# Fro116/RecommenderSystem

Measured on AMD Instinct MI355X. Metric: interactions/sec, higher is better.
Workload: dtype bf16

## Files before the change

include/rsys_debug.h:

```cpp
#ifndef RSYS_DEBUG_H
#define RSYS_DEBUG_H
#include "rsys.h"

#ifdef __cplusplus
extern "C" {
#endif

int32_t rsys_debug_get(rsys_model* m, const char* key, void* out, int64_t bytes);

int32_t rsys_local_group_create(int32_t world, int32_t device, void** group);
int32_t rsys_local_group_destroy(void* group);
int32_t rsys_comm_init_local(void* group, int32_t rank, rsys_comm** out);
int32_t rsys_comm_debug_delay(rsys_comm* c, int32_t microseconds);

int32_t rsys_dev_alloc(void** p, size_t bytes);
int32_t rsys_dev_free(void* p);
int32_t rsys_dev_h2d(void* dst, const void* src, size_t bytes);
int32_t rsys_dev_d2h(void* dst, const void* src, size_t bytes);
int32_t rsys_dev_memset(void* dst, int value, size_t bytes);
int32_t rsys_op_gemm(int32_t dtype, const void* A, const void* B, void* C, int32_t M, int32_t N, int32_t K,
                     int64_t lda, int64_t ldb, int64_t ldc, int32_t a_km, int32_t b_km, int32_t a_f32, int32_t c_f32,
                     int32_t splitk);
int32_t rsys_op_gemm_rows(int32_t dtype, const void* A, const void* B, void* C, int32_t M, int32_t N, int32_t K,
                          int64_t lda, int64_t ldb, int64_t ldc, int32_t b_km, int32_t c_f32, const int32_t* rows_dev);
// ... 7 lines not shown
int32_t rsys_debug_gemm_route(int32_t dtype, int32_t M, int32_t N, int32_t K, int64_t lda, int64_t ldb, int64_t ldc, int32_t a_km,
                              int32_t b_km, int32_t a_f32, int32_t c_f32, int32_t epi, int32_t splitk, int32_t flags, float alpha,
                              int32_t accum, int32_t set, int32_t m_expect, int32_t cus, char* tag, int32_t tag_bytes, int32_t* splits);
int32_t rsys_op_attention(int32_t dtype, int32_t B, int32_t T, int32_t H, int32_t KV, int32_t hd, const void* qkv,
                          const int32_t* uid, const int32_t* tm, void* O, float* lse, const void* dO, void* dqkv,
                          const float* rope_cos, const float* rope_sin);
int32_t rsys_op_attention_ex(int32_t dtype, int32_t B, int32_t T, int32_t H, int32_t KV, int32_t hd, const void* qkv,
                             const int32_t* uid, const int32_t* tm, void* O, float* lse, const void* dO, void* dqkv,
                             const float* rope_cos, const float* rope_sin, const int32_t* rope_pos, int32_t rope_rows,
                             const int32_t* q_active, float* amax_fwd, float* amax_bwd);
int32_t rsys_op_attention_cached(int32_t dtype, int32_t rows, int32_t T, int32_t H, int32_t KV, int32_t hd, const void* qkv, const void* cache,
                                 int32_t n_slots, const int32_t* slot, const int32_t* n_hist, const int32_t* n_cand, void* O);
int32_t rsys_op_attention_cached_tiles(int32_t dtype, int32_t rows, int32_t T, int32_t H, int32_t KV, int32_t hd, const void* qkv, const void* cache,
                                       int32_t n_slots, int32_t Tc, int32_t n_seg, const int32_t* seg, void* O);
int32_t rsys_op_rank_cache_copy_segments(int32_t dtype, int32_t rows, int32_t T, int32_t H, int32_t KV, int32_t hd, const void* qkv, void* cache,
                                         int32_t n_slots, int32_t Tc, int32_t n_seg, const int32_t* seg);
int32_t rsys_rank_cache_get(rsys_model* m, int32_t layer, int32_t slot, void* out, int64_t bytes);
int32_t rsys_op_topk(const float* scores, int64_t ld, int32_t rows, int32_t V, int32_t k,
                     int32_t* ids, float* vals, int32_t* counts);
int32_t rsys_op_target_rank(const float* scores, int64_t ld, int32_t rows, int32_t V, const int32_t* targets, int32_t* rank_out);
int32_t rsys_op_pair_ranks(const float* scores, int64_t ld, int32_t rows, int32_t V, const int32_t* self, const int64_t* tgt_offsets,
                           const int32_t* tgt_ids, int32_t* ranks_out);
int32_t rsys_sim_pair_scores(void* h, int32_t n_src, const int32_t* sources, float* out);
int32_t rsys_rank_gram_get(rsys_model* m, int32_t medium, int32_t n_groups, const int64_t* cand_offsets, const int32_t* cand_ids,
                           float* out, int64_t n_out);
int32_t rsys_op_rerank(int32_t n, int32_t partialk, const float* pen, const float* r, const float* gram, const int32_t* ss_bits,
                       const int32_t* related_bits, int32_t* picks);
int32_t rsys_render_debug_keep(rsys_model* m, int32_t on);
int32_t rsys_render_debug_get(rsys_model* m, const char* key, void* out, int64_t cap, int64_t* bytes);
int32_t rsys_sim_debug_get(void* h, const char* name, void* out, int64_t n);
int32_t rsys_search_debug_get(void* h, const char* name, float* out, int64_t n);
int32_t rsys_op_embedding_scatter(const float* gx0, int64_t ldx, const int32_t* matchedid, const int32_t* m_matchedid, int32_t N,
                                  int32_t V, int32_t D, float* gE, int32_t atomic);
int32_t rsys_op_f8_quantize(const void* src, int64_t ld_src, int32_t rows, int32_t cols, int32_t fmt, int32_t layout, int32_t seg_cols,
                            int32_t seg_rep, void* dst, int64_t ld_dst, float* amax_dev, float* desc_dev, const float* wamax_dev,
                            int32_t n_w, int32_t w_rep, int32_t desc_mode);
int32_t rsys_op_f8_weights(const float* src, int64_t ld, int32_t rows, int32_t cols, int32_t layout, int32_t seg_rows, int32_t seg_rep,
                           float* amax_dev, void* dst, void* dst_t, int64_t ld_t);
int32_t rsys_op_gemm_f8(const void* A8, const void* B8, void* C, int32_t M, int32_t N, int32_t K, int64_t lda, int64_t ldb, int64_t ldc,
                        int32_t a_fmt, int32_t c_f32, const float* desc_dev, int32_t seg_cols, int32_t alt, int32_t kb0, int32_t kb1,
                        int32_t kb2);
int32_t rsys_op_rmsnorm_fwd(int32_t dtype, const float* x, const float* scale, void* y, float* rstd, int64_t rows, int32_t D,
                            const int32_t* rows_dev, const int32_t* in_rows, float* amax);
int32_t rsys_op_rmsnorm_bwd(int32_t dtype, int32_t g_f32, const void* g, const float* x, const float* scale, const float* rstd,
                            const float* resid, const int32_t* resid_slot, const int32_t* io_rows, const int32_t* rows_dev,
                            float* dx, void* dx_t, float* dscale, int64_t rows, int32_t D, float* amax, int32_t deterministic);
int32_t rsys_op_ce(int32_t dtype, void* logits, int64_t ldl, int32_t n, int32_t V, const int32_t* idx, const float* label,
                   const float* weight, const int32_t* position, const float* stats, const int32_t* npos, float task_w, float* loss,
                   int32_t deterministic);
int32_t rsys_op_rating_tail(int32_t dtype, void* z, const void* hact, int32_t n, int32_t D, const float* w2, const float* b2,
                            const int32_t* idx, const float* label, const float* weight, const float* stats, float rating_mean,
                            float task_w, int32_t evaluate, float* loss, float* dw2, float* db2, float* db0, const int32_t* npos,
                            int32_t deterministic);
int32_t rsys_op_sumsq(const float* g, int64_t n, float* out);
int32_t rsys_op_clip_adamw(int32_t dtype, float* p, float* g, float* m, float* v, void* shadow, int64_t n_decay, int64_t n_total,
                           float lr, float b1, float b2, float eps, float wd, int32_t step, float max_norm, float grad_div,
                           int32_t zero_grad, int64_t sh_skip_lo, int64_t sh_skip_hi, int32_t fused, float* sumsq);
int32_t rsys_op_adapter_bank(int32_t dtype, int32_t stages, int32_t train, int32_t rows, int32_t Ttok, int32_t D, int32_t H, int32_t KV, int32_t hd,
                             int32_t L, int32_t layer, float p, uint64_t seed, int64_t stream, const int32_t* row_slot, const void* bankA,
                             const void* bankB, const void* xn, void* La, void* qkv, const void* dqkv, void* dLa, void* dxn, float* partA, float* partB,
                             float* gA, float* gB, const float* rope_cos, const float* rope_sin, const int32_t* rope_pos, int32_t rope_rows);
int32_t rsys_op_adapter_bank_tiles(int32_t dtype, int32_t stages, int32_t rows, int32_t Ttok, int32_t D, int32_t H, int32_t KV, int32_t hd, int32_t L,
                                   int32_t layer, const int32_t* tile_slot, const void* bankA, const void* bankB, const void* xn, void* La, void* qkv,
                                   const float* rope_cos, const float* rope_sin, const int32_t* rope_pos, int32_t rope_rows);
int32_t rsys_op_adapter_bank_segments(int32_t dtype, int32_t stages, int32_t train, int32_t rows, int32_t Ttok, int32_t D, int32_t H, int32_t KV, int32_t hd,
                                      int32_t L, int32_t layer, float p, uint64_t seed, int64_t stream, const int32_t* segs, int32_t n_seg, const void* bankA,
                                      const void* bankB, const void* xn, void* La, void* qkv, const void* dqkv, void* dLa, void* dxn, float* partA,
                                      float* partB, float* gA, float* gB, const float* rope_cos, const float* rope_sin, const int32_t* rope_pos,
                                      int32_t rope_rows);
int32_t rsys_op_adapter_bank_adamw(int32_t dtype, float* A32, float* B32, float* gA, float* gB, float* mA, float* vA, float* mB, float* vB, void* A,
                                   void* B, int64_t nA, int64_t nB, const float* per_slot, float b1, float b2, float eps, float wd, float* norms);
int32_t rsys_op_dropout(int32_t dtype, const void* src, void* dst, int64_t n, float p, uint64_t seed, int64_t stream, int32_t accumulate);
int32_t rsys_op_vp_ce(int32_t dtype, int32_t stages, int32_t deterministic, const int32_t* idx, const float* label, const float* weight,
                      const int32_t* position, const float* stats, const int32_t* npos, float task_w, int32_t KB, int32_t KBmax, float* own,
                      const void* EwAll, const float* metaAll, int32_t W, int32_t D, void* EwC, float* metaC, int32_t* nlive, int32_t* pre,
                      void* logits, int64_t ldl, int32_t Vloc, int32_t col0, float* lmax, const float* gmax, float* sums, int32_t cap,
                      int32_t rank, float* loss, int32_t rows, int32_t rows_finish);
int32_t rsys_op_ss(int32_t dtype, int32_t stages, int32_t deterministic, int32_t len, int32_t n_s, int32_t n_tot, int32_t col0, uint64_t seed,
                   int64_t stream, int32_t* cols, int32_t* bitmap, int32_t* tlist, int32_t* tcount, const float* metaC, const int32_t* nlive,
                   const int32_t* pre, int32_t rank, int32_t cap_rows, int32_t rows, int32_t rows_finish, const void* EwC, const void* Floc,
                   int32_t D, void* logits, int64_t ldl, float* lmax, float* lsum, float* tl, float* gmax, float* loss, float* dt,
                   float* gE_loc, float* dEwC, const int32_t* ridx, int32_t rbase, int64_t rld, int32_t rn, int32_t rtable_rows,
                   const void* gsrc, void* gdst, const float* asrc, float* adst);
int32_t rsys_op_shard_rows(int32_t stages, const int32_t* skey, const int32_t* sidx, int32_t N, int32_t V, int32_t* slot, int32_t* uniq,
                           int32_t* tok2u, int32_t* plan, const int32_t* bound, int32_t nb, int32_t* off, float* table, int64_t ld,
                           int32_t table_rows, const int32_t* ids, int32_t sub, float* packed, int32_t n, int32_t D, const int32_t* count,
                           const int32_t* m_matchedid, const int32_t* userid, const int32_t* m_tmid, int32_t Ntok, const float* Frem,
                           int32_t frem_rows, float* x0, int32_t* uid_t, int32_t* tm_t);

#ifdef __cplusplus
}
#endif
#endif
```

recommendersystem_amd/_lib.py:

```python
import ctypes as C
import os

os.environ.setdefault("HSA_ENABLE_IPC_MODE_LEGACY", "0")

HERE = os.path.dirname(os.path.abspath(__file__))
LIB_PATH = os.path.join(HERE, "librsys_hip.so")


class RsysError(RuntimeError):
    pass


class rsys_config(C.Structure):
    _fields_ = [
        ("num_layers", C.c_int32), ("num_heads", C.c_int32), ("num_kv_heads", C.c_int32),
        ("embed_dim", C.c_int32), ("intermediate_dim", C.c_int32), ("max_sequence_length", C.c_int32),
        ("vocab_0", C.c_int32), ("vocab_1", C.c_int32),
        ("vocab_status", C.c_int32), ("vocab_gender", C.c_int32), ("vocab_source", C.c_int32),
        ("metadata_dim", C.c_int32),
        ("min_ts", C.c_double), ("max_ts", C.c_double),
        ("rating_mean", C.c_float), ("rating_std", C.c_float), ("mask_rate", C.c_float),
        ("mask_topk", C.c_int32), ("finetune", C.c_int32), ("finetune_metric", C.c_int32),
        ("dtype", C.c_int32), ("max_rows", C.c_int32), ("lora_dropout", C.c_float),
        ("table_shard_rank", C.c_int32), ("table_shard_world", C.c_int32), ("sampled_negatives", C.c_int32),
# ... 148 lines not shown
    ("rsys_comm_init", C.c_int32, [C.POINTER(C.c_uint8 * 128), C.c_int32, C.c_int32, C.c_int32, C.POINTER(_P)]),
    ("rsys_comm_destroy", C.c_int32, [_P]),
    ("rsys_comm_debug_delay", C.c_int32, [_P, C.c_int32]),
    ("rsys_set_grad_sync", C.c_int32, [_P, _P]),
    ("rsys_model_set_split_table_reduce", C.c_int32, [_P, C.c_int32]),
    ("rsys_model_set_shard_comm", C.c_int32, [_P, _P]),
    ("rsys_table_rows", C.c_int32, [_P, C.POINTER(C.c_int64), C.POINTER(C.c_int64)]),
    ("rsys_local_group_create", C.c_int32, [C.c_int32, C.c_int32, C.POINTER(_P)]),
    ("rsys_local_group_destroy", C.c_int32, [_P]),
    ("rsys_comm_init_local", C.c_int32, [_P, C.c_int32, C.POINTER(_P)]),
    ("rsys_allreduce_grads", C.c_int32, [_P, _P]),
    ("rsys_grad_sync_early", C.c_int32, [_P, C.POINTER(C.c_int64)]),
    ("rsys_grad_sync_schedule", C.c_int32, [_P, C.POINTER(C.c_int64), C.c_int32, C.POINTER(C.c_int32)]),
    ("rsys_comm_info", C.c_int32, [_P, C.POINTER(C.c_int32)]),
    ("rsys_allreduce_f64", C.c_int32, [_P, C.POINTER(C.c_double), C.c_int32]),
    ("rsys_self_test", C.c_int32, [_P]),
    ("rsys_param_checksum", C.c_int32, [_P, C.POINTER(C.c_double * 4)]),
    ("rsys_grad_buffer", C.c_int32, [_P, C.POINTER(_P), C.POINTER(C.c_int64)]),
    ("rsys_param_buffer", C.c_int32, [_P, C.POINTER(_P), C.POINTER(C.c_int64)]),
    ("rsys_refresh_shadow", C.c_int32, [_P]),
    ("rsys_dev_alloc", C.c_int32, [C.POINTER(_P), C.c_size_t]),
    ("rsys_dev_free", C.c_int32, [_P]),
    ("rsys_dev_h2d", C.c_int32, [_P, _P, C.c_size_t]),
    ("rsys_dev_d2h", C.c_int32, [_P, _P, C.c_size_t]),
    ("rsys_dev_memset", C.c_int32, [_P, C.c_int, C.c_size_t]),
    ("rsys_op_gemm", C.c_int32, [C.c_int32, _P, _P, _P, C.c_int32, C.c_int32, C.c_int32, C.c_int64, C.c_int64, C.c_int64,
                                 C.c_int32, C.c_int32, C.c_int32, C.c_int32, C.c_int32]),
    ("rsys_op_f8_quantize", C.c_int32, [_P, C.c_int64, C.c_int32, C.c_int32, C.c_int32, C.c_int32, C.c_int32, C.c_int32, _P, C.c_int64, _P, _P, _P,
                                          C.c_int32, C.c_int32, C.c_int32]),
    ("rsys_op_f8_weights", C.c_int32, [_P, C.c_int64, C.c_int32, C.c_int32, C.c_int32, C.c_int32, C.c_int32, _P, _P, _P, C.c_int64]),
    ("rsys_op_gemm_f8", C.c_int32, [_P, _P, _P, C.c_int32, C.c_int32, C.c_int32, C.c_int64, C.c_int64, C.c_int64, C.c_int32, C.c_int32, _P,
                                      C.c_int32, C.c_int32, C.c_int32, C.c_int32, C.c_int32]),
    ("rsys_op_gemm_rows", C.c_int32, [C.c_int32, _P, _P, _P, C.c_int32, C.c_int32, C.c_int32, C.c_int64, C.c_int64, C.c_int64,
                                      C.c_int32, C.c_int32, _P]),
    ("rsys_op_gemm_klimit", C.c_int32, [C.c_int32, _P, _P, _P, C.c_int32, C.c_int32, C.c_int32, C.c_int64, C.c_int64, C.c_int64, C.c_int32, _P]),
    ("rsys_op_gemm_epi", C.c_int32, [C.c_int32, _P, _P, _P, C.c_int32, C.c_int32, C.c_int32, C.c_int64, C.c_int64, C.c_int64, C.c_int32, C.c_int32,
                                     C.c_int32, C.c_float, C.c_int32, _P, _P, C.c_int64, _P, C.c_int64, _P, _P, _P, _P, _P,
                                     C.c_int32, C.c_int32, C.c_int32, C.c_int32, _P, C.c_char_p, C.c_int32, C.POINTER(C.c_int32)]),
    ("rsys_debug_gemm_route", C.c_int32, [C.c_int32] * 4 + [C.c_int64] * 3 + [C.c_int32] * 7 + [C.c_float] + [C.c_int32] * 4
                                          + [C.c_char_p, C.c_int32, C.POINTER(C.c_int32)]),
    ("rsys_op_attention", C.c_int32, [C.c_int32] + [C.c_int32] * 5 + [_P] * 9),
    ("rsys_op_attention_ex", C.c_int32, [C.c_int32] + [C.c_int32] * 5 + [_P] * 10 + [C.c_int32, _P, _P, _P]),
    ("rsys_op_topk", C.c_int32, [_P, C.c_int64, C.c_int32, C.c_int32, C.c_int32, _P, _P, _P]),
    ("rsys_op_target_rank", C.c_int32, [_P, C.c_int64, C.c_int32, C.c_int32, _P, _P]),
    ("rsys_op_pair_ranks", C.c_int32, [_P, C.c_int64, C.c_int32, C.c_int32, _P, _P, _P, _P]),
    ("rsys_rank_gram_get", C.c_int32, [_P, C.c_int32, C.c_int32, _P, _P, _P, C.c_int64]),
    ("rsys_op_rerank", C.c_int32, [C.c_int32, C.c_int32, _P, _P, _P, _P, _P, _P]),
    ("rsys_op_embedding_scatter", C.c_int32, [_P, C.c_int64, _P, _P, C.c_int32, C.c_int32, C.c_int32, _P, C.c_int32]),
    ("rsys_op_rmsnorm_fwd", C.c_int32, [C.c_int32, _P, _P, _P, _P, C.c_int64, C.c_int32, _P, _P, _P]),
    ("rsys_op_rmsnorm_bwd", C.c_int32, [C.c_int32, C.c_int32] + [_P] * 11 + [C.c_int64, C.c_int32, _P, C.c_int32]),
    ("rsys_op_ce", C.c_int32, [C.c_int32, _P, C.c_int64, C.c_int32, C.c_int32] + [_P] * 6 + [C.c_float, _P, C.c_int32]),
    ("rsys_op_rating_tail", C.c_int32, [C.c_int32, _P, _P, C.c_int32, C.c_int32] + [_P] * 6 + [C.c_float, C.c_float, C.c_int32]
                                        + [_P] * 5 + [C.c_int32]),
    ("rsys_op_sumsq", C.c_int32, [_P, C.c_int64, _P]),
    ("rsys_op_clip_adamw", C.c_int32, [C.c_int32] + [_P] * 5 + [C.c_int64, C.c_int64] + [C.c_float] * 5
                                       + [C.c_int32, C.c_float, C.c_float, C.c_int32, C.c_int64, C.c_int64, C.c_int32, _P]),
    ("rsys_op_adapter_bank", C.c_int32, [C.c_int32] * 11 + [C.c_float, C.c_uint64, C.c_int64] + [_P] * 16 + [C.c_int32]),
    ("rsys_op_adapter_bank_tiles", C.c_int32, [C.c_int32] * 10 + [_P] * 9 + [C.c_int32]),
    ("rsys_op_adapter_bank_segments", C.c_int32, [C.c_int32] * 11 + [C.c_float, C.c_uint64, C.c_int64, _P, C.c_int32] + [_P] * 15 + [C.c_int32]),
    ("rsys_op_adapter_bank_adamw", C.c_int32, [C.c_int32] + [_P] * 10 + [C.c_int64, C.c_int64, _P] + [C.c_float] * 4 + [_P]),
    ("rsys_op_dropout", C.c_int32, [C.c_int32, _P, _P, C.c_int64, C.c_float, C.c_uint64, C.c_int64, C.c_int32]),
    ("rsys_op_vp_ce", C.c_int32, [C.c_int32] * 3 + [_P] * 6 + [C.c_float, C.c_int32, C.c_int32, _P, _P, _P, C.c_int32, C.c_int32]
                                  + [_P] * 5 + [C.c_int64, C.c_int32, C.c_int32, _P, _P, _P, C.c_int32, C.c_int32, _P, C.c_int32, C.c_int32]),
    ("rsys_op_ss", C.c_int32, [C.c_int32] * 7 + [C.c_uint64, C.c_int64] + [_P] * 7 + [C.c_int32] * 4 + [_P, _P, C.c_int32, _P, C.c_int64]
                               + [_P] * 9 + [C.c_int32, C.c_int64, C.c_int32, C.c_int32] + [_P] * 4),
    ("rsys_op_shard_rows", C.c_int32, [C.c_int32, _P, _P, C.c_int32, C.c_int32] + [_P] * 5 + [C.c_int32, _P, _P, C.c_int64, C.c_int32, _P,
                                       C.c_int32, _P, C.c_int32, C.c_int32] + [_P] * 4 + [C.c_int32, _P, C.c_int32, _P, _P, _P]),
    ("rsys_step_mark", C.c_int32, [_P]),
    ("rsys_step_marks_get", C.c_int32, [_P, _P, C.c_int32, C.POINTER(C.c_int32)]),
    ("rsys_op_timing", C.c_int32, [_P, C.c_int32]),
    ("rsys_timing_get", C.c_int32, [_P, C.c_char_p, C.c_size_t]),
    ("rsys_op_timing_filter", C.c_int32, [_P, C.c_char_p]),
    ("rsys_switches_reload", C.c_int32, []),
    ("rsys_switches_describe", C.c_int32, [C.c_char_p, C.c_int32]),
]
EXPORTED = [s[0] for s in _SIGS]

_lib = None


def lib():
    global _lib
    if _lib is None:
        if not os.path.exists(LIB_PATH):
            raise RsysError(f"{LIB_PATH} is missing: build it with `make -C recommendersystem_amd/csrc` "
                            "(there is no CPU fallback for the HIP path)")
        L = C.CDLL(LIB_PATH, mode=C.RTLD_GLOBAL)
        for name, res, args in _SIGS:
            fn = getattr(L, name)
            fn.restype = res
            fn.argtypes = args
        _lib = L
    return _lib


def last_error():
    buf = C.create_string_buffer(2048)
    lib().rsys_last_error(buf, 2048)
    return buf.value.decode(errors="replace")


def check(rc):
    if rc != 0:
        raise RsysError(f"rsys error {rc}: {last_error()}")


# ... 17 lines not shown
```

recommendersystem_amd/csrc/capi.hip:

```cpp
#include <algorithm>
#include <dlfcn.h>
#include <math.h>
#include <stdlib.h>
#include <string.h>

#include <sstream>

#include "comm.hpp"
#include "encoder_handle.hpp"
#include "model_internal.hpp"

namespace rsys {
static thread_local std::string g_err;
void set_error(const std::string& msg) { g_err = msg; }
}

using namespace rsys;

struct rsys_model { Model* m; };
struct rsys_optimizer { Optimizer o; };

#define CHECK_HANDLE(h) do { if ((h) == nullptr) { set_error("null handle"); return RSYS_ERR_ARG; } } while (0)

extern "C" {
// ... 1136 lines not shown
int32_t rsys_op_rmsnorm_bwd(int32_t dtype, int32_t g_f32, const void* g, const float* x, const float* scale, const float* rstd,
                            const float* resid, const int32_t* resid_slot, const int32_t* io_rows, const int32_t* rows_dev,
                            float* dx, void* dx_t, float* dscale, int64_t rows, int32_t D, float* amax, int32_t deterministic) {
  switches_parse();
  ARG_CHECK(g && x && scale && rstd && dx && dscale && rows >= 0, "rsys_op_rmsnorm_bwd: arguments");
  ARG_CHECK(!g_f32 || (resid_slot == nullptr && io_rows == nullptr), "rsys_op_rmsnorm_bwd: the f32-gradient form takes no resid_slot / io_rows");
  HookDet det(deterministic != 0);
  const long long wgs = std::max<long long>(1, std::min<long long>(rows, 4LL * std::max(1, sw().debug_norm_bwd_grid)));
  RC(det.alloc(wgs * D, ceil32(wgs) * D));
  const bool bf = dtype == RSYS_DTYPE_BF16;
  int rc;
  if (g_f32) rc = bf ? launch_rmsnorm_bwd_f32<bf16>((const float*)g, x, scale, rstd, resid, dx, (bf16*)dx_t, dscale, rows, D, nullptr, rows_dev, amax)
                     : launch_rmsnorm_bwd_f32<float>((const float*)g, x, scale, rstd, resid, dx, (float*)dx_t, dscale, rows, D, nullptr, rows_dev, amax);
  else rc = bf ? launch_rmsnorm_bwd<bf16>((const bf16*)g, x, scale, rstd, resid, dx, (bf16*)dx_t, dscale, rows, D, nullptr, rows_dev, resid_slot, io_rows, amax)
               : launch_rmsnorm_bwd<float>((const float*)g, x, scale, rstd, resid, dx, (float*)dx_t, dscale, rows, D, nullptr, rows_dev, resid_slot, io_rows, amax);
  if (rc) return rc;
  HIP_CHECK(hipDeviceSynchronize());
  return det.check("rsys_op_rmsnorm_bwd");
}

int32_t rsys_op_ce(int32_t dtype, void* logits, int64_t ldl, int32_t n, int32_t V, const int32_t* idx, const float* label,
                   const float* weight, const int32_t* position, const float* stats, const int32_t* npos, float task_w, float* loss,
                   int32_t deterministic) {
  switches_parse();
  ARG_CHECK(logits && idx && label && weight && position && stats && loss && n >= 0 && V >= 1, "rsys_op_ce: arguments");
  HookDet det(deterministic != 0 && n > 0);
  RC(det.alloc(n, ceil32(n)));
  int rc = dtype == RSYS_DTYPE_BF16 ? launch_ce_fwd_bwd<bf16>((bf16*)logits, ldl, n, V, idx, label, weight, position, stats, npos, task_w, loss, nullptr)
                                    : launch_ce_fwd_bwd<float>((float*)logits, ldl, n, V, idx, label, weight, position, stats, npos, task_w, loss, nullptr);
  if (rc) return rc;
  HIP_CHECK(hipDeviceSynchronize());
  return det.check("rsys_op_ce");
}

int32_t rsys_op_rating_tail(int32_t dtype, void* z, const void* hact, int32_t n, int32_t D, const float* w2, const float* b2,
                            const int32_t* idx, const float* label, const float* weight, const float* stats, float rating_mean,
                            float task_w, int32_t evaluate, float* loss, float* dw2, float* db2, float* db0, const int32_t* npos,
                            int32_t deterministic) {
  switches_parse();
  ARG_CHECK(z && hact && w2 && b2 && idx && label && weight && stats && loss && dw2 && db2 && db0 && n >= 0, "rsys_op_rating_tail: arguments");
  HookDet det(deterministic != 0 && n > 0);
  const long long grid = std::min<long long>((n + 3) / 4, 512);
  RC(det.alloc(grid * (2LL * D + 4), ceil32(grid) * D));
  int rc = dtype == RSYS_DTYPE_BF16
               ? launch_rating_tail<bf16>((bf16*)z, (const bf16*)hact, n, D, w2, b2, idx, label, weight, stats, rating_mean, task_w, evaluate, loss,
                                          dw2, db2, db0, nullptr, npos)
               : launch_rating_tail<float>((float*)z, (const float*)hact, n, D, w2, b2, idx, label, weight, stats, rating_mean, task_w, evaluate, loss,
                                           dw2, db2, db0, nullptr, npos);
  if (rc) return rc;
  HIP_CHECK(hipDeviceSynchronize());
  return det.check("rsys_op_rating_tail");
}

int32_t rsys_op_sumsq(const float* g, int64_t n, float* out) {
  ARG_CHECK(g && out, "rsys_op_sumsq: arguments");
  float* part = nullptr;
  HIP_CHECK(hipMalloc((void**)&part, (size_t)sumsq_parts() * 4));
  int rc = launch_sumsq(g, n, out, part, nullptr, true);
  hipError_t e = hipDeviceSynchronize();
  hipFree(part);
  if (rc) return rc;
  HIP_CHECK(e);
  return RSYS_OK;
}

int32_t rsys_op_clip_adamw(int32_t dtype, float* p, float* g, float* m, float* v, void* shadow, int64_t n_decay, int64_t n_total,
                           float lr, float b1, float b2, float eps, float wd, int32_t step, float max_norm, float grad_div,
                           int32_t zero_grad, int64_t sh_skip_lo, int64_t sh_skip_hi, int32_t fused, float* sumsq) {
  switches_parse();
  ARG_CHECK(p && g && m && v && sumsq && n_total >= 4 && step >= 1, "rsys_op_clip_adamw: arguments");
  float* part = nullptr;
  HIP_CHECK(hipMalloc((void**)&part, (size_t)sumsq_parts() * 4));
  const bool bf = dtype == RSYS_DTYPE_BF16;
  int rc = launch_sumsq(g, n_total, sumsq, part, nullptr, true);
  if (fused) {
    const float* ss = max_norm > 0.f ? sumsq : nullptr;
    if (!rc) rc = bf ? launch_adamw<bf16>(p, g, m, v, (bf16*)shadow, n_decay, n_total, lr, b1, b2, eps, wd, step, ss, grad_div, max_norm, zero_grad, nullptr,
                                          sh_skip_lo, sh_skip_hi)
                     : launch_adamw<float>(p, g, m, v, nullptr, n_decay, n_total, lr, b1, b2, eps, wd, step, ss, grad_div, max_norm, zero_grad, nullptr);
  } else {
    if (!rc) rc = launch_scale(g, n_total, sumsq, grad_div, max_norm, nullptr);
    if (!rc) rc = bf ? launch_adamw<bf16>(p, g, m, v, (bf16*)shadow, n_decay, n_total, lr, b1, b2, eps, wd, step, nullptr, 1.f, 0.f, zero_grad, nullptr,
                                          sh_skip_lo, sh_skip_hi)
                     : launch_adamw<float>(p, g, m, v, nullptr, n_decay, n_total, lr, b1, b2, eps, wd, step, nullptr, 1.f, 0.f, zero_grad, nullptr);
  }
  hipError_t e = hipDeviceSynchronize();
  hipFree(part);
  if (rc) return rc;
  HIP_CHECK(e);
  return RSYS_OK;
}

int32_t rsys_op_adapter_bank(int32_t dtype, int32_t stages, int32_t train, int32_t rows, int32_t Ttok, int32_t D, int32_t H, int32_t KV, int32_t hd,
                             int32_t L, int32_t layer, float p, uint64_t seed, int64_t stream, const int32_t* row_slot, const void* bankA,
                             const void* bankB, const void* xn, void* La, void* qkv, const void* dqkv, void* dLa, void* dxn, float* partA, float* partB,
                             float* gA, float* gB, const float* rope_cos, const float* rope_sin, const int32_t* rope_pos, int32_t rope_rows) {
  switches_parse();
  return adapter_bank_op(dtype, stages, train, rows, Ttok, D, H, KV, hd, L, layer, p, seed, stream, row_slot, bankA, bankB, xn, La, qkv, dqkv, dLa, dxn,
                         partA, partB, gA, gB, rope_cos, rope_sin, rope_pos, rope_rows);
}

int32_t rsys_op_adapter_bank_tiles(int32_t dtype, int32_t stages, int32_t rows, int32_t Ttok, int32_t D, int32_t H, int32_t KV, int32_t hd, int32_t L,
                                   int32_t layer, const int32_t* tile_slot, const void* bankA, const void* bankB, const void* xn, void* La, void* qkv,
                                   const float* rope_cos, const float* rope_sin, const int32_t* rope_pos, int32_t rope_rows) {
  switches_parse();
  return adapter_bank_op(dtype, stages, 0, rows, Ttok, D, H, KV, hd, L, layer, 0.f, 0, 0, tile_slot, bankA, bankB, xn, La, qkv, nullptr, nullptr, nullptr,
// ... 287 lines not shown
```

recommendersystem_amd/csrc/elementwise.hip:

```cpp
#include "kernels.hpp"

namespace rsys {

thread_local DetScratch g_det;

__global__ void reduce_parts_kernel(const float* __restrict__ part, int nparts, long long stride, int n, float* dst) {
  const int c = blockIdx.x * blockDim.x + threadIdx.x;
  if (c >= n) return;
  float acc = 0.f;
  for (int b = 0; b < nparts; ++b) acc += part[(long long)b * stride + c];
  dst[c] += acc;
}
__global__ void reduce_parts_stage_kernel(const float* __restrict__ part, int nparts, long long stride, int n, float* out) {
  const int c = blockIdx.x * blockDim.x + threadIdx.x, chunk = blockIdx.y;
  if (c >= n) return;
  const int b0 = chunk * 32, b1 = min(nparts, b0 + 32);
  float acc = 0.f;
  for (int b = b0; b < b1; ++b) acc += part[(long long)b * stride + c];
  out[(long long)chunk * n + c] = acc;
}
int launch_reduce_parts(const float* part, int nparts, long long stride, int n, float* dst, hipStream_t s) {
  if (nparts <= 0 || n <= 0) return RSYS_OK;
  if (nparts > 64 && g_det.tmp != nullptr) {
    const int chunks = (nparts + 31) / 32;
// ... 662 lines not shown
  for (int c = threadIdx.x; c < nacc; c += 256) sds[c] = 0.f;
  __syncthreads();
  float* const mine = part != nullptr ? sds + w * 2 * D : sds;
  float l0 = 0.f, l1 = 0.f, l2 = 0.f, gb2 = 0.f;
  const float inv_ws = 1.f / fmaxf(stats[0], 1e-8f);
  if (npos != nullptr) n = min(n, (*npos + 127) & ~127);
  for (int row = blockIdx.x * 4 + w; row < n; row += gridDim.x * 4) {
    const int i = idx[row];
    const float wt = weight[i], tgt = label[i] - rating_mean;
    const T* hr = hact + (long long)row * D;
    T* zr = z + (long long)row * D;
    float acc = 0.f;
    for (int c = l; c < D; c += 64) acc += to_f32(hr[c]) * w2[c];
    acc = wave_sum(acc);
    const float pred = acc + b2[0];
    const float e1 = pred - tgt;
    l0 += e1 * e1 * wt; l1 += tgt * tgt * wt; l2 += (-pred - tgt) * (-pred - tgt) * wt;
    const float dpred = evaluate ? 0.f : task_w * 2.f * e1 * wt * inv_ws;
    gb2 += dpred;
    for (int c = l; c < D; c += 64) {
      float zz = to_f32(zr[c]);
      float gp = 0.5f * (1.f + erff(zz * 0.70710678118654752f)) + zz * __expf(-0.5f * zz * zz) * 0.3989422804014327f;
      float dz = dpred * w2[c] * gp;
      zr[c] = from_f32<T>(dz);
      if (dpred != 0.f) {
        if (part != nullptr) { mine[c] += dpred * to_f32(hr[c]); mine[D + c] += dz; }
        else { atomicAdd(&sds[c], dpred * to_f32(hr[c])); atomicAdd(&sds[D + c], dz); }
      }
    }
  }
  if (part != nullptr) {
    float* sc = sds + 4 * 2 * D;
    if (l == 0) { sc[w * 4 + 0] = gb2; sc[w * 4 + 1] = l0; sc[w * 4 + 2] = l1; sc[w * 4 + 3] = l2; }
    __syncthreads();
    float* pr = part + (long long)blockIdx.x * (2 * D + 4);
    for (int c = threadIdx.x; c < 2 * D; c += 256) pr[c] = ((sds[c] + sds[2 * D + c]) + sds[4 * D + c]) + sds[6 * D + c];
    if (threadIdx.x < 4) pr[2 * D + threadIdx.x] = ((sc[threadIdx.x] + sc[4 + threadIdx.x]) + sc[8 + threadIdx.x]) + sc[12 + threadIdx.x];
    return;
  }
  __syncthreads();
  if (!evaluate) {
    for (int c = threadIdx.x; c < D; c += 256) {
      if (sds[c] != 0.f) atomicAdd(&dw2[c], sds[c]);
      if (sds[D + c] != 0.f) atomicAdd(&db0[c], sds[D + c]);
    }
    if (l == 0 && gb2 != 0.f) atomicAdd(db2, gb2);
  }
  if (l == 0) {
    if (l0 != 0.f) atomicAdd(&loss_out[0], l0);
    if (l1 != 0.f) atomicAdd(&loss_out[1], l1);
    if (l2 != 0.f) atomicAdd(&loss_out[2], l2);
  }
}
template <typename T>
int launch_rating_tail(T* z, const T* hact, int n, int D, const float* w2, const float* b2, const int* idx,
                       const float* label, const float* weight, const float* stats, float rating_mean, float task_w,
                       int evaluate, float* loss_out, float* dw2, float* db2, float* db0, hipStream_t s, const int* npos) {
  if (n <= 0) return RSYS_OK;
  int grid = std::min(div_up(n, 4), 512);
  const long long prow = 2LL * D + 4;
  float* part = det_part(grid * prow);
  hipLaunchKernelGGL((rating_tail_kernel<T>), dim3(grid), dim3(256), (part ? 8 * D + 16 : 2 * D) * sizeof(float), s, z, hact, n, D, w2, b2, idx,
                     label, weight, stats, rating_mean, task_w, evaluate, loss_out, dw2, db2, db0, part, npos);
  HIP_CHECK(hipGetLastError());
  if (part != nullptr) {
    int rc = RSYS_OK;
    if (!evaluate) {
      rc = launch_reduce_parts(part, grid, prow, D, dw2, s);
      if (rc == RSYS_OK) rc = launch_reduce_parts(part + D, grid, prow, D, db0, s);
      if (rc == RSYS_OK) rc = launch_reduce_parts(part + 2 * D, grid, prow, 1, db2, s);
    }
    return rc == RSYS_OK ? launch_reduce_parts(part + 2 * D + 1, grid, prow, 3, loss_out, s) : rc;
  }
  return RSYS_OK;
}
template int launch_rating_tail<bf16>(bf16*, const bf16*, int, int, const float*, const float*, const int*, const float*, const float*, const float*, float, float, int, float*, float*, float*, float*, hipStream_t, const int*);
template int launch_rating_tail<float>(float*, const float*, int, int, const float*, const float*, const int*, const float*, const float*, const float*, float, float, int, float*, float*, float*, float*, hipStream_t, const int*);

template <typename T>
__global__ void widen_kernel(const T* __restrict__ src, float* __restrict__ dst, long long n) {
  for (long long i = (long long)blockIdx.x * blockDim.x + threadIdx.x; i < n; i += (long long)gridDim.x * blockDim.x) dst[i] = to_f32(src[i]);
}
template <typename T>
int launch_widen(const T* src, float* dst, long long n, hipStream_t s) {
  const int blocks = (int)std::min<long long>((n + 255) / 256, 8192);
  hipLaunchKernelGGL((widen_kernel<T>), dim3(blocks), dim3(256), 0, s, src, dst, n);
  HIP_CHECK(hipGetLastError());
  return RSYS_OK;
}
template int launch_widen<bf16>(const bf16*, float*, long long, hipStream_t);
template int launch_widen<float>(const float*, float*, long long, hipStream_t);
template <typename T>
__global__ void rowdot_kernel(const T* __restrict__ h, const float* __restrict__ w, const float* __restrict__ b, float* out, int n, int D) {
  const int row = (blockIdx.x * blockDim.x + threadIdx.x) >> 6, l = threadIdx.x & 63;
  if (row >= n) return;
  const T* hr = h + (long long)row * D;
  float acc = 0.f;
  for (int c = l; c < D; c += 64) acc += to_f32(hr[c]) * w[c];
  acc = wave_sum(acc);
  if (l == 0) out[row] = acc + b[0];
}
template <typename T>
int launch_rowdot(const T* h, const float* w, const float* b, float* out, int n, int D, hipStream_t s) {
  hipLaunchKernelGGL((rowdot_kernel<T>), dim3(div_up(n, 4)), dim3(256), 0, s, h, w, b, out, n, D);
  HIP_CHECK(hipGetLastError());
  return RSYS_OK;
}
template int launch_rowdot<bf16>(const bf16*, const float*, const float*, float*, int, int, hipStream_t);
template int launch_rowdot<float>(const float*, const float*, const float*, float*, int, int, hipStream_t);

template <typename TS>
__global__ void colsum_kernel(const TS* __restrict__ src, long long ld, long long rows, int cols, float* dst, int rows_per_block, float* part) {
  const int c = blockIdx.x * blockDim.x + threadIdx.x;
  if (c >= cols) return;
  const long long r0 = (long long)blockIdx.y * rows_per_block, r1 = min(rows, r0 + rows_per_block);
  float acc = 0.f;
  for (long long r = r0; r < r1; ++r) acc += to_f32(src[r * ld + c]);
  if (part != nullptr) part[(long long)blockIdx.y * cols + c] = acc;
  else if (acc != 0.f) atomicAdd(&dst[c], acc);
}
template <typename TS>
static int colsum_any(const TS* src, long long ld, long long rows, int cols, float* dst, hipStream_t s) {
  int rpb = (int)std::max<long long>(64, (rows + 511) / 512);
  dim3 grid(div_up(cols, 256), div_up(rows, rpb));
  float* part = det_part((long long)grid.y * cols);
  hipLaunchKernelGGL((colsum_kernel<TS>), grid, dim3(256), 0, s, src, ld, rows, cols, dst, rpb, part);
  HIP_CHECK(hipGetLastError());
  if (part != nullptr) return launch_reduce_parts(part, (int)grid.y, cols, cols, dst, s);
  return RSYS_OK;
}
int launch_colsum_add(const float* src, long long ld, long long rows, int cols, float* dst, hipStream_t s) {
  return colsum_any<float>(src, ld, rows, cols, dst, s);
}

__global__ __launch_bounds__(1024) void cast_colsum_kernel(const float* __restrict__ src, bf16* __restrict__ dst, long long rows, int D,
                                                           float* colsum, int rows_per_block, float* part) {
  __shared__ float red[2048];
  const int cg = D >> 2;
  const int c = (threadIdx.x % cg) * 4, lane_r = threadIdx.x / cg, nr = 1024 / cg;
  const long long r0 = (long long)blockIdx.x * rows_per_block, r1 = min(rows, r0 + rows_per_block);
  float4 acc = make_float4(0, 0, 0, 0);
  long long r = r0 + lane_r;
  for (; r + 3 * nr < r1; r += 4 * nr) {
    float4 v[4];
#pragma unroll
    for (int u = 0; u < 4; ++u) v[u] = *(const float4*)(src + (r + u * nr) * D + c);
#pragma unroll
    for (int u = 0; u < 4; ++u) {
      bf16x4 o; o[0] = (bf16)v[u].x; o[1] = (bf16)v[u].y; o[2] = (bf16)v[u].z; o[3] = (bf16)v[u].w;
      *(bf16x4*)(dst + (r + u * nr) * D + c) = o;
      acc.x += v[u].x; acc.y += v[u].y; acc.z += v[u].z; acc.w += v[u].w;
    }
  }
  for (; r < r1; r += nr) {
    const float4 v = *(const float4*)(src + r * D + c);
    bf16x4 o; o[0] = (bf16)v.x; o[1] = (bf16)v.y; o[2] = (bf16)v.z; o[3] = (bf16)v.w;
    *(bf16x4*)(dst + r * D + c) = o;
    acc.x += v.x; acc.y += v.y; acc.z += v.z; acc.w += v.w;
  }
  if (lane_r < 2) *(float4*)&red[lane_r * D + c] = acc;
  __syncthreads();
  for (int base = 2; base < nr; base += 2) {
    if (lane_r >= base && lane_r < base + 2) {
      float4 o = *(float4*)&red[(lane_r - base) * D + c];
      o.x += acc.x; o.y += acc.y; o.z += acc.z; o.w += acc.w;
      *(float4*)&red[(lane_r - base) * D + c] = o;
    }
    __syncthreads();
  }
  for (int cc = threadIdx.x; cc < D; cc += 1024) {
    const float v = red[cc] + (nr > 1 ? red[D + cc] : 0.f);
    if (part != nullptr) part[(long long)blockIdx.x * D + cc] = v;
    else if (v != 0.f) atomicAdd(&colsum[cc], v);
  }
}
int launch_cast_colsum(const float* src, bf16* dst, long long rows, int D, float* colsum, hipStream_t s) {
  ARG_CHECK(D % 4 == 0 && D <= 1024 && 1024 % (D >> 2) == 0, "cast_colsum: D/4 must divide 1024, D <= 1024");
  const int rpb = (int)std::max<long long>(32, (rows + 511) / 512);
  const int grid = div_up(rows, rpb);
  float* part = det_part((long long)grid * D);
  hipLaunchKernelGGL(cast_colsum_kernel, dim3(grid), dim3(1024), 0, s, src, dst, rows, D, colsum, rpb, part);
  HIP_CHECK(hipGetLastError());
  if (part != nullptr) return launch_reduce_parts(part, grid, D, D, colsum, s);
  return RSYS_OK;
// ... 159 lines not shown
```

recommendersystem_amd/csrc/kernels.hpp:

```cpp
#pragma once
#include "common.hpp"

namespace rsys {

struct BatchDev {
  int N, rows, S;
  const int *userid, *tmid, *gender, *source, *matchedid, *status;
  const double* time;
  const float *rating, *progress;
  const float* label[6]; const float* weight[6]; const int* position[6];
  const unsigned char *watch_mask, *rating_mask;
  const int* rope_pos;
  int *m_tmid, *m_matchedid, *m_status;
  float *m_rating, *m_progress;
  float* m_label[4]; float* m_weight[4]; int* m_position[4];
};

struct DetScratch {
  float* part = nullptr; long long cap = 0; float* tmp = nullptr; long long tmp_cap = 0;
  int part_used = 0, part_short = 0;
};
extern thread_local DetScratch g_det;
int launch_reduce_parts(const float* part, int nparts, long long stride, int n, float* dst, hipStream_t s);

// ... 9 lines not shown
                       unsigned long long seed, unsigned long long step, hipStream_t s);

int launch_mask_tokens_rows(BatchDev b, const int* row_task, hipStream_t s);
int launch_mask_tokens_tiles(BatchDev b, const int* tile_task, hipStream_t s);

template <typename T>
int launch_action_features(const BatchDev& b, const SmallParams& sp, T* feat , hipStream_t s);

int launch_gather_items(const BatchDev& b, const float* F32, int V, int D, float* x0, int* uid_t, int* tm_t, hipStream_t s);

template <typename T>
int launch_rmsnorm_fwd(const float* x, const float* scale, T* y, float* rstd, long long rows, int D, hipStream_t s, const int* rows_dev = nullptr,
                       const int* in_rows = nullptr ,
                       float* f8_amax = nullptr );

template <typename T>
int launch_rmsnorm_bwd(const T* g, const float* x, const float* scale, const float* rstd, const float* resid_grad,
                       float* dx_out, T* dx_out_t, float* dscale, long long rows, int D, hipStream_t s, const int* rows_dev = nullptr,
                       const int* resid_slot = nullptr ,
                       const int* io_rows = nullptr ,
                       float* f8_amax = nullptr );
template <typename T>
int launch_rmsnorm_bwd_f32(const float* g, const float* x, const float* scale, const float* rstd, const float* resid_grad,
                           float* dx_out, T* dx_out_t, float* dscale, long long rows, int D, hipStream_t s, const int* rows_dev = nullptr,
                           float* f8_amax = nullptr);

template <typename T>
int launch_dropout(const T* src, T* dst, long long n, float p, unsigned long long seed, unsigned int stream, int accumulate, hipStream_t s);

int launch_select_positions(const float* w, int N, int topk, int* idx, float* stats ,
                            int* npos_out , hipStream_t s);
int launch_select_positions_chunked(int ntask, const float* const* w, int N, int topk, int* const* idx, float* const* stats, int* const* npos_out,
                                    void* scratch, hipStream_t s);
int launch_select_positions_batch(int ntask, const float* const* w, int N, int topk, int* const* idx, float* const* stats,
                                  int* const* npos_out, hipStream_t s);

template <typename T>
int launch_gather_rows(const T* src, long long ld, const int* idx, int parity, T* dst, int n, int D, hipStream_t s);

int launch_scatter_rows_add(const float* src, const int* idx, int parity, float* dst, long long ld, int n, int D, hipStream_t s,
                            const int* npos = nullptr );

template <typename T>
int launch_ce_fwd_bwd(T* logits, long long ldl, int n, int V, const int* idx, const float* label, const float* weight,
                      const int* position, const float* stats, const int* npos, float task_w, float* loss_out, hipStream_t s);

template <typename T>
int launch_rating_tail(T* z, const T* hact, int n, int D, const float* w2, const float* b2, const int* idx,
                       const float* label, const float* weight, const float* stats, float rating_mean, float task_w,
                       int evaluate, float* loss_out , float* dw2, float* db2, float* db0, hipStream_t s,
                       const int* npos = nullptr );

int launch_colsum_add(const float* src, long long ld, long long rows, int cols, float* dst, hipStream_t s);
int launch_cast_colsum(const float* src, bf16* dst, long long rows, int D, float* colsum, hipStream_t s);
int launch_cast_transpose_colsum(const float* src, bf16* dstT, long long rows, int D, long long ldt, float* colsum, hipStream_t s);

int launch_embedding_scatter_add(const float* gx0, const BatchDev& b, int V, int D, float* gE, hipStream_t s);

int token_index_capacity(int N);
int launch_token_index_build(const int* matchedid, int N, int V, unsigned long long* keys, int* skey, int* sidx, hipStream_t s);
size_t seg_scatter_slab_floats(int N, int D);
int launch_embedding_scatter_segmented(const float* gx0, long long ldx, const int* m_matchedid, const int* skey, const int* sidx,
                                       int N, int V, int D, float* gE, float* slab, hipStream_t s);

int launch_token_union(const int* const* idx, const int* const* npos, int ntask, int NT, unsigned int* bits, int* pre, int* nsel, hipStream_t s);
int launch_selected_first(const unsigned int* bits, const int* pre, int* slot, int* sel, const int* uid, const int* tm, const int* rope_pos, int B, int T,
                          int* perm, int* uid_p, int* tm_p, int* pos_p, int* slot_p, int* sel_p, int* q_active, hipStream_t s);
template <typename T> int launch_gather_rows_sel(const T* src, long long ld, const int* sel, const int* n_dev, int cap, T* dst, int D, hipStream_t s);
template <typename T> int launch_scatter_rows_fill(const T* src, const int* slot_p, const int* q_active, int B, int Tseq, T* dst, long long ld, int D, hipStream_t s);
template <typename T> int launch_scatter_rows_sel(const T* src, const int* sel, const int* n_dev, int cap, T* dst, long long ld, int D, hipStream_t s);
template <typename T> int launch_scatter_rows_map(const T* src, const int* map, int n, T* dst, long long ld, int D, hipStream_t s);
template <typename T> int launch_gather_rows_slot(const T* compact, const int* slot, const int* idx, int parity, T* dst, int n, int D, hipStream_t s);
int launch_scatter_rows_add_slot(const float* src, const int* slot, const int* idx, int parity, const int* npos, float* compact, int n, int D, hipStream_t s);

int launch_plan_unique(const int* skey, const int* sidx, int N, int V, int* slot, int* uniq, int* tok2u, int* plan , hipStream_t s);
int launch_plan_offsets(const int* uniq, const int* plan, const int* bound_dev, int nb, int* off, hipStream_t s);
int launch_gather_rows_by_id(const float* src, long long ld, const int* ids, int sub, float* dst, int n, int D, hipStream_t s);
int launch_add_rows_by_id(const float* src, const int* ids, int sub, float* dst, long long ld, int n, int D, hipStream_t s);
int launch_add_rows_by_id_counted(const float* src, const int* ids, const int* count_dev, float* dst, long long ld, int cap, int D, hipStream_t s);
int launch_gather_items_remote(const BatchDev& b, const float* Frem, const int* tok2u, const int* plan, int D, float* x0,
                               int* uid_t, int* tm_t, hipStream_t s);
int launch_vp_meta(const int* idx, const float* label, const float* weight, const int* position, const float* stats,
                   const int* npos, float task_w, int KB, int KBmax, float* own , hipStream_t s);
int launch_add_scalar(float* dst, const float* src, hipStream_t s);
template <typename T>
int launch_vp_compact(const T* EwAll, const float* metaAll, int W, int KB, int D, T* EwC, float* metaC, int* nlive, int* pre , hipStream_t s);
template <typename T>
int launch_vp_stats(const T* logits, long long ldl, int Vloc, int col0, const float* metaC, const int* nlive, float* lmax,
                    float* sums , int cap, int grid_rows, hipStream_t s);
int launch_vp_rebase(const float* lmax, const float* gmax, float* sums, int n, hipStream_t s);
template <typename T>
int launch_vp_finish(T* logits, long long ldl, int Vloc, int col0, const float* metaC, const float* gmax, const float* sums, int cap,
                     const int* nlive, const int* pre, int rank, float* loss_out, int grid_rows, hipStream_t s);

int launch_ss_sample(int len, int n_s, unsigned long long seed, unsigned int stream, int* cols, hipStream_t s);
template <typename T> int launch_gather_rows_plain(const T* src, long long ld, const int* idx, int base, T* dst, int n, int D, hipStream_t s);
int launch_add_rows_plain(const float* src, const int* idx, int base, float* dst, long long ld, int n, int D, hipStream_t s);
template <typename T>
int launch_ss_target_logit(const T* EwC, const T* Floc, int D, int len, int col0, const float* metaC, const int* nlive, float* tl, int grid_rows, hipStream_t s);
template <typename T>
int launch_ss_stats(const T* logits, long long ldl, int n_s, int n_tot, int len, int col0, const int* cols, const float* metaC, const int* nlive,
                    float* lmax, float* lsum, int grid_rows, hipStream_t s);
int launch_ss_targets(const float* metaC, const int* nlive, int cap_rows, int len, int col0, unsigned int* bitmap, int* out, int* count, hipStream_t s);
int launch_ss_drop_hits(int* cols, int n_s, const unsigned int* bitmap, hipStream_t s);
int launch_ss_max_with_target(const float* lmax, const float* tl, float* out, int n, hipStream_t s);
int launch_ss_rebase(const float* lmax, const float* gmax, float* lsum, int n, hipStream_t s);
// ... 99 lines not shown
```

Before: 1.618 million.

## Add row-parallel rating tail and vectorized colsum kernels for non-deterministic mode

Adds a rating-tail kernel that gives each wave one row, keeps per-column gradient accumulators in registers, reduces them through shared-memory atomics and then global atomics. It replaces the partial-buffer path when determinism is off. Also adds a float4 column-sum kernel that splits rows across blocks with an in-block tree reduction, replacing the generic colsum, plus a debug entry point to compare both forms. The aim is to cut launch and partial-reduction overhead and memory passes, at the cost of non-deterministic atomic accumulation.

```diff
diff --git a/include/rsys_debug.h b/include/rsys_debug.h
--- a/include/rsys_debug.h
+++ b/include/rsys_debug.h
@@ -83,6 +83,7 @@
                             const int32_t* idx, const float* label, const float* weight, const float* stats, float rating_mean,
                             float task_w, int32_t evaluate, float* loss, float* dw2, float* db2, float* db0, const int32_t* npos,
                             int32_t deterministic);
+int32_t rsys_op_colsum_add(const float* src, int64_t ld, int64_t rows, int32_t cols, float* dst, int32_t scalar_form, int32_t deterministic);
 int32_t rsys_op_sumsq(const float* g, int64_t n, float* out);
 int32_t rsys_op_clip_adamw(int32_t dtype, float* p, float* g, float* m, float* v, void* shadow, int64_t n_decay, int64_t n_total,
                            float lr, float b1, float b2, float eps, float wd, int32_t step, float max_norm, float grad_div,
diff --git a/recommendersystem_amd/_lib.py b/recommendersystem_amd/_lib.py
--- a/recommendersystem_amd/_lib.py
+++ b/recommendersystem_amd/_lib.py
@@ -224,6 +224,7 @@
     ("rsys_op_ce", C.c_int32, [C.c_int32, _P, C.c_int64, C.c_int32, C.c_int32] + [_P] * 6 + [C.c_float, _P, C.c_int32]),
     ("rsys_op_rating_tail", C.c_int32, [C.c_int32, _P, _P, C.c_int32, C.c_int32] + [_P] * 6 + [C.c_float, C.c_float, C.c_int32]
                                         + [_P] * 5 + [C.c_int32]),
+    ("rsys_op_colsum_add", C.c_int32, [_P, C.c_int64, C.c_int64, C.c_int32, _P, C.c_int32, C.c_int32]),
     ("rsys_op_sumsq", C.c_int32, [_P, C.c_int64, _P]),
     ("rsys_op_clip_adamw", C.c_int32, [C.c_int32] + [_P] * 5 + [C.c_int64, C.c_int64] + [C.c_float] * 5
                                        + [C.c_int32, C.c_float, C.c_float, C.c_int32, C.c_int64, C.c_int64, C.c_int32, _P]),
diff --git a/recommendersystem_amd/csrc/capi.hip b/recommendersystem_amd/csrc/capi.hip
--- a/recommendersystem_amd/csrc/capi.hip
+++ b/recommendersystem_amd/csrc/capi.hip
@@ -1212,6 +1212,18 @@
   return det.check("rsys_op_rating_tail");
 }
 
+int32_t rsys_op_colsum_add(const float* src, int64_t ld, int64_t rows, int32_t cols, float* dst, int32_t scalar_form, int32_t deterministic) {
+  switches_parse();
+  ARG_CHECK(src && dst && rows >= 1 && cols >= 1 && ld >= cols, "rsys_op_colsum_add: arguments");
+  HookDet det(deterministic != 0);
+  const long long parts = (rows + 63) / 64;
+  RC(det.alloc(parts * cols, ceil32(parts) * cols));
+  int rc = scalar_form ? launch_colsum_add_scalar(src, ld, rows, cols, dst, nullptr) : launch_colsum_add(src, ld, rows, cols, dst, nullptr);
+  if (rc) return rc;
+  HIP_CHECK(hipDeviceSynchronize());
+  return det.check("rsys_op_colsum_add");
+}
+
 int32_t rsys_op_sumsq(const float* g, int64_t n, float* out) {
   ARG_CHECK(g && out, "rsys_op_sumsq: arguments");
   float* part = nullptr;
diff --git a/recommendersystem_amd/csrc/elementwise.hip b/recommendersystem_amd/csrc/elementwise.hip
--- a/recommendersystem_amd/csrc/elementwise.hip
+++ b/recommendersystem_amd/csrc/elementwise.hip
@@ -738,11 +738,100 @@
     if (l2 != 0.f) atomicAdd(&loss_out[2], l2);
   }
 }
+constexpr int kTailWaves = 4;
+template <typename T, int NJ>
+__global__ __launch_bounds__(64 * kTailWaves) void rating_tail_rows_kernel(T* z, const T* __restrict__ hact, int n, int D,
+                                                                const float* __restrict__ w2, const float* __restrict__ b2,
+                                                                const int* __restrict__ idx, const float* __restrict__ label,
+                                                                const float* __restrict__ weight, const float* __restrict__ stats,
+                                                                float rating_mean, float task_w, int evaluate, float* loss_out,
+                                                                float* dw2, float* db2, float* db0, const int* __restrict__ npos) {
+  extern __shared__ __attribute__((aligned(16))) float sds[];
+  const int l = threadIdx.x & 63, w = threadIdx.x >> 6, nw = blockDim.x >> 6;
+  if (npos != nullptr) n = min(n, (*npos + 127) & ~127);
+  if (blockIdx.x * nw >= n) return;
+  for (int c = threadIdx.x; c < 2 * D + 4; c += blockDim.x) sds[c] = 0.f;
+  __syncthreads();
+  float w2v[NJ], adw[NJ], adb[NJ];
+#pragma unroll
+  for (int j = 0; j < NJ; ++j) { const int c = l + 64 * j; w2v[j] = c < D ? w2[c] : 0.f; adw[j] = 0.f; adb[j] = 0.f; }
+  float l0 = 0.f, l1 = 0.f, l2 = 0.f, gb2 = 0.f;
+  const float inv_ws = 1.f / fmaxf(stats[0], 1e-8f);
+  for (int row = blockIdx.x * nw + w; row < n; row += gridDim.x * nw) {
+    const int i = idx[row];
+    const T* hr = hact + (long long)row * D;
+    T* zr = z + (long long)row * D;
+    float hv[NJ], zv[NJ];
+#pragma unroll
+    for (int j = 0; j < NJ; ++j) {
+      const int c = l + 64 * j;
+      hv[j] = c < D ? to_f32(hr[c]) : 0.f;
+      zv[j] = c < D ? to_f32(zr[c]) : 0.f;
+    }
+    const float wt = weight[i], tgt = label[i] - rating_mean;
+    float acc = 0.f;
+#pragma unroll
+    for (int j = 0; j < NJ; ++j) if (l + 64 * j < D) acc += hv[j] * w2v[j];
+    acc = wave_sum(acc);
+    const float pred = acc + b2[0];
+    const float e1 = pred - tgt;
+    l0 += e1 * e1 * wt; l1 += tgt * tgt * wt; l2 += (-pred - tgt) * (-pred - tgt) * wt;
+    const float dpred = evaluate ? 0.f : task_w * 2.f * e1 * wt * inv_ws;
+    gb2 += dpred;
+#pragma unroll
+    for (int j = 0; j < NJ; ++j) {
+      const int c = l + 64 * j;
+      if (c < D) {
+        const float zz = zv[j];
+        const float gp = 0.5f * (1.f + erff(zz * 0.70710678118654752f)) + zz * __expf(-0.5f * zz * zz) * 0.3989422804014327f;
+        const float dz = dpred * w2v[j] * gp;
+        zr[c] = from_f32<T>(dz);
+        if (dpred != 0.f) { adw[j] += dpred * hv[j]; adb[j] += dz; }
+      }
+    }
+  }
+  if (!evaluate) {
+#pragma unroll
+    for (int j = 0; j < NJ; ++j) {
+      const int c = l + 64 * j;
+      if (c < D && adw[j] != 0.f) atomicAdd(&sds[c], adw[j]);
+      if (c < D && adb[j] != 0.f) atomicAdd(&sds[D + c], adb[j]);
+    }
+  }
+  if (l == 0) {
+    float* sc = sds + 2 * D;
+    if (gb2 != 0.f) atomicAdd(&sc[0], gb2);
+    if (l0 != 0.f) atomicAdd(&sc[1], l0);
+    if (l1 != 0.f) atomicAdd(&sc[2], l1);
+    if (l2 != 0.f) atomicAdd(&sc[3], l2);
+  }
+  __syncthreads();
+  if (!evaluate) {
+    for (int c = threadIdx.x; c < D; c += blockDim.x) {
+      if (sds[c] != 0.f) atomicAdd(&dw2[c], sds[c]);
+      if (sds[D + c] != 0.f) atomicAdd(&db0[c], sds[D + c]);
+    }
+    if (threadIdx.x == 0 && sds[2 * D] != 0.f) atomicAdd(db2, sds[2 * D]);
+  }
+  if (threadIdx.x < 3 && sds[2 * D + 1 + threadIdx.x] != 0.f) atomicAdd(&loss_out[threadIdx.x], sds[2 * D + 1 + threadIdx.x]);
+}
 template <typename T>
 int launch_rating_tail(T* z, const T* hact, int n, int D, const float* w2, const float* b2, const int* idx,
                        const float* label, const float* weight, const float* stats, float rating_mean, float task_w,
                        int evaluate, float* loss_out, float* dw2, float* db2, float* db0, hipStream_t s, const int* npos) {
   if (n <= 0) return RSYS_OK;
+  if (g_det.part == nullptr && D <= 1024) {
+    const dim3 g(std::min(div_up(n, kTailWaves), 4096 / kTailWaves)), b(64 * kTailWaves);
+    const size_t lds = (2 * D + 4) * sizeof(float);
+#define RSYS_TAIL_ROWS(NJ) hipLaunchKernelGGL((rating_tail_rows_kernel<T, NJ>), g, b, lds, s, z, hact, n, D, w2, b2, idx, label, weight, stats, \
+                                              rating_mean, task_w, evaluate, loss_out, dw2, db2, db0, npos)
+    if (D <= 128) RSYS_TAIL_ROWS(2);
+    else if (D <= 512) RSYS_TAIL_ROWS(8);
+    else RSYS_TAIL_ROWS(16);
+#undef RSYS_TAIL_ROWS
+    HIP_CHECK(hipGetLastError());
+    return RSYS_OK;
+  }
   int grid = std::min(div_up(n, 4), 512);
   const long long prow = 2LL * D + 4;
   float* part = det_part(grid * prow);
@@ -815,7 +904,55 @@
   if (part != nullptr) return launch_reduce_parts(part, (int)grid.y, cols, cols, dst, s);
   return RSYS_OK;
 }
+__global__ __launch_bounds__(1024) void colsum_rows_kernel(const float* __restrict__ src, long long ld, long long rows, int cols, float* dst, int rows_per_block) {
+  __shared__ float4 red[1024];
+  const int cg = cols >> 2, nr = 1024 / cg;
+  const int ci = threadIdx.x % cg, lane_r = threadIdx.x / cg;
+  if (lane_r < nr) {
+    const float* col = src + ci * 4;
+    const long long r0 = (long long)blockIdx.x * rows_per_block, r1 = min(rows, r0 + rows_per_block);
+    float4 acc = make_float4(0, 0, 0, 0);
+    long long r = r0 + lane_r;
+    for (; r + 3 * nr < r1; r += 4 * nr) {
+      float4 v[4];
+#pragma unroll
+      for (int u = 0; u < 4; ++u) v[u] = *(const float4*)(col + (r + u * nr) * ld);
+#pragma unroll
+      for (int u = 0; u < 4; ++u) { acc.x += v[u].x; acc.y += v[u].y; acc.z += v[u].z; acc.w += v[u].w; }
+    }
+    for (; r < r1; r += nr) {
+      const float4 v = *(const float4*)(col + r * ld);
+      acc.x += v.x; acc.y += v.y; acc.z += v.z; acc.w += v.w;
+    }
+    red[lane_r * cg + ci] = acc;
+  }
+  __syncthreads();
+  int h = 1;
+  while (h < nr) h <<= 1;
+  for (h >>= 1; h >= 1; h >>= 1) {
+    if (lane_r < h && lane_r + h < nr) {
+      float4 a = red[lane_r * cg + ci];
+      const float4 b = red[(lane_r + h) * cg + ci];
+      a.x += b.x; a.y += b.y; a.z += b.z; a.w += b.w;
+      red[lane_r * cg + ci] = a;
+    }
+    __syncthreads();
+  }
+  const float* sum = (const float*)red;
+  for (int cc = threadIdx.x; cc < cols; cc += 1024)
+    if (sum[cc] != 0.f) atomicAdd(&dst[cc], sum[cc]);
+}
+int launch_colsum_add_scalar(const float* src, long long ld, long long rows, int cols, float* dst, hipStream_t s) {
+  return colsum_any<float>(src, ld, rows, cols, dst, s);
+}
 int launch_colsum_add(const float* src, long long ld, long long rows, int cols, float* dst, hipStream_t s) {
+  const bool rows16 = cols % 4 == 0 && cols >= 4 && cols <= 4096 && ld % 4 == 0 && ((uintptr_t)src & 15) == 0;
+  if (g_det.part == nullptr && rows16 && rows > 0) {
+    const int rpb = (int)std::max<long long>(256, (rows + 127) / 128);
+    hipLaunchKernelGGL(colsum_rows_kernel, dim3(div_up(rows, rpb)), dim3(1024), 0, s, src, ld, rows, cols, dst, rpb);
+    HIP_CHECK(hipGetLastError());
+    return RSYS_OK;
+  }
   return colsum_any<float>(src, ld, rows, cols, dst, s);
 }
 
diff --git a/recommendersystem_amd/csrc/kernels.hpp b/recommendersystem_amd/csrc/kernels.hpp
--- a/recommendersystem_amd/csrc/kernels.hpp
+++ b/recommendersystem_amd/csrc/kernels.hpp
@@ -85,6 +85,7 @@
                        const int* npos = nullptr );
 
 int launch_colsum_add(const float* src, long long ld, long long rows, int cols, float* dst, hipStream_t s);
+int launch_colsum_add_scalar(const float* src, long long ld, long long rows, int cols, float* dst, hipStream_t s);
 int launch_cast_colsum(const float* src, bf16* dst, long long rows, int D, float* colsum, hipStream_t s);
 int launch_cast_transpose_colsum(const float* src, bf16* dstT, long long rows, int D, long long ldt, float* colsum, hipStream_t s);
 
```

New measurement: 1.627 million (median of 6 runs). No clear change (+0.6%).
